# CompVis/unsupervised-part-segmentation

Hardware: AMD Instinct MI355X
Metric: images/sec training (CUB 128x128, 10 parts) (higher is better)
Workload: dtype bf16

## Files before the change

### include/upsparts_hip.h

```cpp
#ifndef UPSPARTS_HIP_H
#define UPSPARTS_HIP_H

#include <stddef.h>
#include <stdint.h>

#ifdef __cplusplus
extern "C" {
#endif

#define UPS_ABI_VERSION 6

enum { UPS_F32 = 0, UPS_BF16 = 1, UPS_F16 = 2 };
enum { UPS_ACT_NONE = 0, UPS_ACT_LRELU = 1, UPS_ACT_RELU = 2, UPS_ACT_ELU = 3 };
enum { UPS_OK = 0, UPS_E_ARG = -1, UPS_E_UNSUPPORTED = -2, UPS_E_LAUNCH = -3 };

int ups_abi_version(void);
void ups_struct_sizes(int64_t out[4]);
const char* ups_last_error(void);

typedef struct {
    int32_t dtype;
    int32_t n, hi, wi;
    int32_t ci;
    int32_t ldi;
// ... 25 lines not shown
    float*       mask_grad;
    const float* mask_view;
    const float* f8_deq;
    const float* f8_scale;
    float*       f8_amax;
    int32_t      f8_e5m2;
    const void*  in_f8;
    void*        out_f8;
    const float* out_f8_scale;
    float*       out_f8_amax;
    int32_t      out_f8_act, out_f8_e5m2;
    int32_t      d2s;
    int32_t      out_act, res_act;
    void*        sign_out;
    const void*  dact_bits;
} ups_conv_desc;

int ups_conv_igemm(const ups_conv_desc* d, void* stream);
int ups_conv_sign_out_written(void);

int ups_weight_prep_d2s(const float* src, int32_t cin_v, int32_t ci_log, int32_t co, int32_t pad_y, int32_t pad_x, int32_t C,
                        void* w, void* stream);

int ups_weight_prep_f8(const float* src, int32_t ntaps, int32_t cin_v, int32_t ci_log, int32_t co, int32_t transpose,
                       void* w_f8, float* deq, void* stream);

typedef struct {
    int32_t dtype;
    int32_t n, hi, wi, ci, ldi;
    int32_t ci_log;
    int32_t cin_v;
    int32_t ho, wo, co, ldo;
    int32_t in_sy, in_sx;
    int32_t ntaps;
    int32_t tap_dy[9], tap_dx[9], tap_w[9];
    int32_t act_in; float act_slope;
    int32_t splitk;
// ... 250 lines not shown
```

### unsupervised-part-segmentation_amd/csrc/common.h

```cpp
#pragma once
#include <hip/hip_runtime.h>
#include <stdint.h>
#include <stdio.h>
#include <type_traits>

#include "../../include/upsparts_hip.h"
#include "env.h"

typedef __bf16 bf16;
typedef __attribute__((ext_vector_type(8))) __bf16 bf16x8;
typedef _Float16 f16;
typedef __attribute__((ext_vector_type(8))) _Float16 f16x8;
typedef __attribute__((ext_vector_type(2))) _Float16 f16x2;
typedef __attribute__((ext_vector_type(4))) short s16x4;
typedef __attribute__((ext_vector_type(4))) float f32x4;
typedef __attribute__((ext_vector_type(16))) float f32x16;

void ups_set_error(const char* fmt, ...);

extern thread_local int g_ups_sign_written;

struct UpsPerDevice {
    unsigned long long bits = 0;
    static int cur() { int d = 0; (void)hipGetDevice(&d); return d & 63; }
// ... 233 lines not shown

__device__ inline float block_sum_256(float v, float* smem4) {
    v = wave_sum(v);
    const int lane = threadIdx.x & 63, wid = threadIdx.x >> 6;
    __syncthreads();
    if (lane == 0) smem4[wid] = v;
    __syncthreads();
    return smem4[0] + smem4[1] + smem4[2] + smem4[3];
}

__device__ __forceinline__ void ups_amax_slot(float* slot, float m) {
    if (m > __builtin_nontemporal_load(slot)) atomicMax((unsigned*)slot, __float_as_uint(m));
}

static inline int ups_cdiv(long long a, long long b) { return (int)((a + b - 1) / b); }
```

### unsupervised-part-segmentation_amd/csrc/conv3x3_patch.hip

```cpp
#include <stdlib.h>

#include "common.h"

namespace {

constexpr int TS = 16;
constexpr int PW = TS + 2;
constexpr int PPIX = PW * PW;
constexpr int RS = 80;
constexpr int PWP = 20;
constexpr int APX = 64;
constexpr int A_BYTES = PW * PWP * APX;
__device__ __forceinline__ int a_swz(int px) { return (px >> 2) & 3; }
__device__ __forceinline__ int a_swz16(int px) { return ((px >> 2) & 1) << 1; }
template <typename T> __device__ __forceinline__ int a_swz_t(int px) { return sizeof(T) == 2 ? a_swz16(px) : a_swz(px); }

template <int V> struct IC { static constexpr int value = V; };

struct PatchK {
    int n, h, w, ci, ldi, co, co_fill, ldo, ldr, ldd, act_in, out_f32, dact_kind, has_ctab;
    float act_slope;
    unsigned long long tap_off, tap_wi;
    const void* in; const void* wgt; void* out;
    const float* bias; const float* coord_tab; const void* res; const void* dact;
    unsigned char* sign_out; const unsigned char* dact_bits;
    const unsigned* mask; float* mask_grad; const float* mask_view;
    int mask_B, mask_P;
    unsigned m_ntn, m_parts, m_tx, m_ty;
    const float* f8_deq; const float* f8_scale; float* f8_amax;
    int f8_e5m2;
    const unsigned char* in_f8; unsigned char* out_f8; const float* out_f8_scale; float* out_f8_amax;
    int out_f8_act, out_f8_e5m2;
    int d2s, d2s_shift;
    int taps_static;
    int out_act, res_act;
    int res_patch;
    int sgn_off;
    int sgn_res;
};

__device__ __forceinline__ int fast_div(int n, int d, unsigned m) {
    if (d == 1) return n;
    return m ? (int)__umulhi((unsigned)n, m) : n / d;
}
static inline unsigned div_magic(long long n_max, int d) {
    if (d <= 1 || n_max * d >= (1ll << 32)) return 0u;
    return (unsigned)(((1ull << 32) + (unsigned)d - 1) / (unsigned)d);
}
// ... 49 lines not shown
                        acc[i][2 * jh + jj] = __builtin_amdgcn_mfma_f32_16x16x32_fp8_bf8(fb[step & 1][jj][1], fa[i][1], acc[i][2 * jh + jj], 0, 0, 0);
                    } else if constexpr (F8 == 1) {
                        acc[i][2 * jh + jj] = __builtin_amdgcn_mfma_f32_16x16x32_fp8_fp8(fb[step & 1][jj][0], fa[i][0], acc[i][2 * jh + jj], 0, 0, 0);
                        acc[i][2 * jh + jj] = __builtin_amdgcn_mfma_f32_16x16x32_fp8_fp8(fb[step & 1][jj][1], fa[i][1], acc[i][2 * jh + jj], 0, 0, 0);
                    } else if constexpr (sizeof(T) == 2 && !__is_same(T, bf16)) {
                        acc[i][2 * jh + jj] = __builtin_amdgcn_mfma_f32_16x16x32_f16(fb[step & 1][jj], fa[i], acc[i][2 * jh + jj], 0, 0, 0);
                    } else {
                        acc[i][2 * jh + jj] = __builtin_amdgcn_mfma_f32_16x16x32_bf16(fb[step & 1][jj], fa[i], acc[i][2 * jh + jj], 0, 0, 0);
                    }
            __builtin_amdgcn_s_setprio(0);
            if (jh + 1 == NP && t + 1 < 3) fetch_a(t + 1);
        }
    }
}

typedef __attribute__((ext_vector_type(8))) int i32x8v;
template <int TM16, int TN16, int ROWB, int ABYTES, int BHALF, bool E5M2, int BBUFS>
__device__ __forceinline__ void f8s_tap(const unsigned char* A, const unsigned char* B, int at, f32x4v (&acc)[TM16][TN16]) {
    typedef __attribute__((ext_vector_type(4))) int i32x4v;
    i32x8v fa[TM16], fb[BBUFS];
    auto cat = [](i32x4v lo, i32x4v hi) __attribute__((always_inline)) -> i32x8v {
        return __builtin_shufflevector(lo, hi, 0, 1, 2, 3, 4, 5, 6, 7);
    };
    auto fetch_b = [&](int j, int slot) __attribute__((always_inline)) {
        fb[slot] = cat(*(const i32x4v*)(B + j * (16 * 64)), *(const i32x4v*)(B + BHALF + j * (16 * 64)));
    };
    fetch_b(0, 0);
#pragma unroll
    for (int i = 0; i < TM16; ++i) fa[i] = cat(*(const i32x4v*)(A + at + i * ROWB), *(const i32x4v*)(A + ABYTES + at + i * ROWB));
#pragma unroll
// ... 38 lines not shown
                                                                     acc[i][j], 0, 0, 0);
    }
};

template <typename T, int BN, int OCC, int SUB, int F8 = 0, bool PRE = false, int TAPS = 0, bool DMAP = false, bool CSTD = false>
__global__ __launch_bounds__(512, 2 * OCC) void conv3x3_patch_kernel(const PatchK p, const int tiles_x, const int tiles_y,
                                                                 const int ntn, const int kchunks, const int nblocks) {
    constexpr int EPC = Chunk<T>::N;
    constexpr int BK = 4 * EPC;
    constexpr int BKA = F8 ? 64 : BK;
    constexpr bool F8S = F8 >= 3;
    constexpr int F8K = F8S ? F8 - 2 : F8;
    static_assert(!F8 || (sizeof(T) == 2 && SUB == TS && (OCC == 1 || PRE)), "fp8 operands: bf16 tensors, one tile per image; two blocks per CU only with a pre-quantised input");
    static_assert(!F8S || (PRE && OCC == 2 && BN >= 64 && TAPS == 0 && !DMAP), "block-scaled fp8: pre-quantised input, two blocks per CU");
    static_assert(!PRE || F8, "a pre-quantised input implies fp8 operands");
    constexpr int WN = (BN == 32) ? 1 : 2;
    constexpr int WM = 8 / WN;
    constexpr int TM = 256 / WM / 32;
    constexpr int TN = BN / WN / 32;
    constexpr int B_BYTES = 3 * BN * RS;
    constexpr int NB = (3 * BN * 4 + 511) / 512;
    constexpr int HALF_OFF = (sizeof(T) == 2) ? 16 : 32;
    constexpr int G = TS / SUB;
    constexpr int PR = G * (SUB + 2);
    constexpr int PWPS = (PR + 3) / 4 * 4;
    constexpr int ABY = PR * PWPS * APX;
    static_assert(SUB == 16 || OCC == 1, "multi-image tiles run one block per CU");

    extern __shared__ __attribute__((aligned(16))) unsigned char smem[];
    unsigned char* Abuf = smem;
// ... 217 lines not shown
    const int r = lane & 31, hh = lane >> 5;
    const int ty_l = (wm * TM * 2) + (r >> 4), tx_l = r & 15;
    const int py_l = ty_l + 2 * (ty_l / SUB) * (SUB < TS ? 1 : 0), px_l = tx_l + 2 * (tx_l / SUB) * (SUB < TS ? 1 : 0);
    const int a_lane_off = (py_l * PWPS + px_l) * APX;
    const int b_lane_off = (wn * TN * 32 + r) * RS + hh * HALF_OFF;
    const int p16 = lane & 15, q16 = lane >> 4;
    const int px_l16 = p16 + 2 * (p16 / SUB) * (SUB < TS ? 1 : 0);
    const int a_lane16 = px_l16 * APX;
    int arow16[TM16];
#pragma unroll
    for (int i = 0; i < TM16; ++i) {
        const int ty = wm * TM16 + i;
        arow16[i] = (ty + 2 * (ty / SUB) * (SUB < TS ? 1 : 0)) * PWPS * APX;
    }

    const int total = 3 * kchunks;
    if constexpr (sizeof(T) == 2) {
        constexpr int BST = 3 * BN * 64;
        constexpr int NJ = 3 * BN * 4 / 64;
        constexpr int NW = (NJ + 7) / 8;
        constexpr bool CHUNKST = (SUB < TS || (CSTD && DMAP && SUB == TS)) && BN <= 64 && F8 == 0 && OCC == 1;
        constexpr int NST = (OCC == 2) ? 2 : (CHUNKST ? 6 : 3);
        constexpr int FRAG_BUFS = (BN == 128) ? 1 : 2;
        unsigned char* Bst = smem + (((kchunks == 1 && SUB == TS) || OCC == 2) ? 1 : 2) * ABY;
        const int boff16 = p16 * 64 + ((q16 ^ a_swz16(p16)) << 4);
        int d_tl[NW];
        unsigned d_off[NW];
#pragma unroll
        for (int q = 0; q < NW; ++q) {
            const int j = (wid + 8 * q) % NJ;
            const int pos = j * 64 + lane, row = pos >> 2, slot = pos & 3;
            const int tl = (j * 16) / BN, rl = row - tl * BN;
            const int c = min(nt * BN + rl, p.co - 1);
            d_tl[q] = tl;
            d_off[q] = (unsigned)(c * BK + (slot ^ a_swz16(row)) * 8) * 2u;
        }
        const unsigned smem_lds = (unsigned)(unsigned long long)(__attribute__((address_space(3))) unsigned char*)smem;
        auto dma_w = [&](int it) __attribute__((always_inline)) {
            const int cc = it / 3, g = it - cc * 3;
            unsigned char* stg = Bst + (it % NST) * BST;
#pragma unroll
            for (int q = 0; q < NW; ++q) {
                const int j = (wid + 8 * q) % NJ;
                const int wslice = TAPS != 0 ? 3 * g + d_tl[q] : p_w(p.tap_wi, 3 * g + d_tl[q]);
                const T* slab = w + ((long long)wslice * kchunks + cc) * p.co * BK;
                const unsigned lds_dst = __builtin_amdgcn_readfirstlane(smem_lds + (unsigned)(stg + j * 1024 - smem));
                asm volatile("s_mov_b32 m0, %0\n\ts_nop 0\n\tglobal_load_lds_dwordx4 %1, %2"
                             :: "s"(lds_dst), "v"(d_off[q]), "s"(slab) : "memory", "m0");
            }
        };
        const unsigned char* __restrict__ in_b = (const unsigned char*)(in + (long long)origin * p.ldi);
        auto dma_patch = [&](int cc, int boff = 0) __attribute__((always_inline)) {
            if constexpr (DMAP) {
                const unsigned char* base = in_b + cc * 64;
#pragma unroll
                for (int q = 0; q < 3; ++q) {
                    if (wid + 8 * q >= (PW * PWPS + 15) / 16) continue;
                    const unsigned lds_dst = __builtin_amdgcn_readfirstlane(smem_lds + (unsigned)(boff + (wid + 8 * q) * 1024));
                    asm volatile("s_mov_b64 exec, %0\n\ts_mov_b32 m0, %1\n\ts_nop 0\n\tglobal_load_lds_dwordx4 %2, %3\n\ts_mov_b64 exec, -1"
                                 :: "s"(pd_mask[q]), "s"(lds_dst), "v"(pd_off[q]), "s"(base) : "memory", "m0");
                }
            }
        };
        const int swx0 = a_lane16 + ((q16 ^ a_swz16(px_l16 + 0)) << 4);
        const int swx1 = a_lane16 + ((q16 ^ a_swz16(px_l16 + 1)) << 4);
        const int swx2 = a_lane16 + ((q16 ^ a_swz16(px_l16 + 2)) << 4);
        constexpr int CPW = TN16 / 2 > 0 ? TN16 / 2 : 1;
        const int rp_first = nt * (BN / 32) + wn * CPW;
        const int rp_lane = ((px_l16 + 1) * APX) + ((((q16 >> 1)) ^ a_swz16(px_l16 + 1)) << 4) + (q16 & 1) * 8;
        constexpr bool RP2 = DMAP && SUB == TS && TN16 >= 2 && TAPS == 2 && BN == 128 && F8 == 0 && __is_same(T, bf16);
        const unsigned char* S1 = smem + p.sgn_off;
        const float rp2_inv = (RP2 && p.res_patch == 2) ? 1.f / dact_ns : 1.f;
        auto add_res_patch = [&](const unsigned char* A, int cc) __attribute__((always_inline)) {
            if constexpr (DMAP && SUB == TS && TN16 >= 2) {
                const int c2 = cc - rp_first;
                if (p.res_patch && c2 >= 0 && c2 < CPW) {
                    int ln = lane;
                    if constexpr (RP2) asm volatile("" : "+v"(ln));
                    const int sg_lane = (ln & 15) * (BN / 8) + (ln >> 5), sg_sh = (ln >> 2) & 4;
#pragma unroll
                    for (int jh = 0; jh < CPW; ++jh) {
// ... 94 lines not shown
            const unsigned char* row = p.dact_bits + (((long long)img_pm * p.h + yy) * p.w + xx) * (p.ldd >> 3) + boff;
            if (yy < p.h && xx < p.w) {
                if (RP2 || (SG_BPP >= 8 && rem >= 8)) sgn_v = *(const uint2*)row;
                else if (rem >= 4) sgn_v.x = *(const unsigned*)row;
            }
        }
        if constexpr (DMAP) dma_patch(0);
        else { load_patch(0); store_patch(Abuf); }
        dma_w(0);
        if (sgn_on && sgn_px < 256) {
            if constexpr (SG_BPP >= 8) *(uint2*)(smem + p.sgn_off + sgn_px * SG_BPP + 8 * sgn_hf) = sgn_v;
            else *(unsigned*)(smem + p.sgn_off + sgn_px * SG_BPP) = sgn_v.x;
        }
        if (OCC != 2 && total > 1) dma_w(1);
        const bool one_shot = OCC != 2 && kchunks == 1;
        if (one_shot || CHUNKST) dma_w(2);
        asm volatile("s_waitcnt vmcnt(0)" ::: "memory");
        __syncthreads();
        if (one_shot) {
            add_res_patch(Abuf, 0);
#pragma unroll
            for (int g = 0; g < 3; ++g) {
                const unsigned char* B = Bst + g * BST + (wn * TN * 32) * 64 + boff16;
                if constexpr (TAPS != 0) {
                    const int po0 = ((TAPS == 1 ? g : 2 - g) * PWPS + (TAPS == 1 ? 0 : 2)) * APX;
                    bf16_taps16<T, TM16, TN16, (SUB == TS ? PWPS * APX : 0), F8>(Abuf, B, arow16, po0, po0 + (TAPS == 1 ? APX : -APX),
                                            po0 + (TAPS == 1 ? 2 * APX : -2 * APX), TAPS == 1 ? swx0 : swx2, swx1, TAPS == 1 ? swx2 : swx0,
                                            BN * 64, acc16);
                } else {
                    const int dx0 = p_dx(p.tap_off, 3 * g) + 1, dx1 = p_dx(p.tap_off, 3 * g + 1) + 1, dx2 = p_dx(p.tap_off, 3 * g + 2) + 1;
                    const int po0 = ((p_dy(p.tap_off, 3 * g) + 1) * PWPS + dx0) * APX;
                    const int po1 = ((p_dy(p.tap_off, 3 * g + 1) + 1) * PWPS + dx1) * APX;
                    const int po2 = ((p_dy(p.tap_off, 3 * g + 2) + 1) * PWPS + dx2) * APX;
// ... 492 lines not shown
        "conv3x3_patch_kernel", (epi > shmem_max ? epi : shmem_max) + sgn_bytes, dim3(nblocks), dim3(512), shmem, s, kk, tiles_x, tiles_y, ntn,
        kchunks, nblocks);
}

template <typename T, int SUB>
int launch_small(const PatchK& k, hipStream_t s) {
    const int tiles = k.n / ((TS / SUB) * (TS / SUB));
    if (k.co_fill > 64 && tiles * ups_cdiv(k.co_fill, 128) >= 192) return launch_bn<T, 128, 1, SUB>(k, s);
    if (k.co_fill > 32 && tiles * ups_cdiv(k.co_fill, 64) >= 128) return launch_bn<T, 64, 1, SUB>(k, s);
    return launch_bn<T, 32, 1, SUB>(k, s);
}

template <typename T, int BN, int OCC>
int launch_v(const PatchK& k, hipStream_t s) {
    const bool dmap = k.act_in == UPS_ACT_NONE && !k.mask && !k.mask_grad && k.ci % 32 == 0;
    if (dmap) {
        if (k.taps_static == 1) return launch_bn<T, BN, OCC, TS, 0, false, 1, true>(k, s);
        if (k.taps_static == 2) return launch_bn<T, BN, OCC, TS, 0, false, 2, true>(k, s);
    }
    if (k.taps_static == 1 && BN == 128 && OCC == 2) return launch_bn<T, BN, OCC, TS, 0, false, (BN == 128 && OCC == 2) ? 1 : 0>(k, s);
    return launch_bn<T, BN, OCC, TS>(k, s);
}

template <typename T>
int launch_t(const PatchK& k, hipStream_t s) {
    if (k.h == 8) return launch_small<T, 8>(k, s);
    if (k.h == 4) return launch_small<T, 4>(k, s);
    if constexpr (sizeof(T) == 2) {
      if constexpr (__is_same(T, bf16)) {
        if (k.f8_deq && k.in_f8) {
// ... 19 lines not shown
            }
            if (k.co_fill > 64) return launch_bn<T, 128, 1, TS, 1>(k, s);
            if (k.co_fill > 32) return launch_bn<T, 64, 1, TS, 1>(k, s);
            return launch_bn<T, 32, 1, TS, 1>(k, s);
        }
      }
        const int tiles = k.n * ((k.w + TS - 1) / TS) * ((k.h + TS - 1) / TS);
        if (k.co_fill > 64 && k.ci > 32) {
            if (!k.out_f8_amax && tiles * ups_cdiv(k.co_fill, 128) >= 512) return launch_v<T, 128, 2>(k, s);
            if (tiles * ups_cdiv(k.co_fill, 64) >= 512) return launch_v<T, 64, 2>(k, s);
            {
                const bool dmap = k.act_in == UPS_ACT_NONE && !k.mask && !k.mask_grad && k.ci % 32 == 0;
                if (dmap && !k.out_f8_amax && k.ci >= 128 && tiles * ups_cdiv(k.co_fill, 128) <= 256) {
                    if (k.taps_static == 1) return launch_bn<T, 64, 1, TS, 0, false, 1, true, true>(k, s);
                    if (k.taps_static == 2) return launch_bn<T, 64, 1, TS, 0, false, 2, true, true>(k, s);
                }
            }
            return launch_v<T, 128, 1>(k, s);
        }
        if (k.co_fill > 32) {
            if (k.co_fill > 64 && tiles * ups_cdiv(k.co_fill, 128) >= 512) {
                if (k.out_f8_amax) return launch_bn<T, 128, 2, TS>(k, s);
                return launch_v<T, 128, 2>(k, s);
            }
            return (k.ci > 32 && tiles * ups_cdiv(k.co_fill, 64) >= 512) ? launch_v<T, 64, 2>(k, s) : launch_v<T, 64, 1>(k, s);
        }
        return launch_v<T, 32, 1>(k, s);
    } else {
        if (k.co_fill > 64) return launch_bn<T, 128, 1, TS>(k, s);
        if (k.co_fill > 32) return launch_bn<T, 64, 1, TS>(k, s);
// ... 32 lines not shown
        seen[(dy + 1) * 3 + dx + 1] = true;
    }
    for (int t = 0; t < 9; ++t) if (!seen[t]) return 1;
    if (d->coord_tab) {
        for (int t = 0; t < 9; ++t) if (d->tap_dy[t] != t / 3 - 1 || d->tap_dx[t] != t % 3 - 1) return 1;
    }
    PatchK k;
    k.mask = d->mask_bits; k.mask_grad = d->mask_grad; k.mask_view = d->mask_view;
    k.f8_deq = d->f8_deq; k.f8_scale = d->f8_scale; k.f8_amax = d->f8_amax; k.f8_e5m2 = d->f8_e5m2;
    k.in_f8 = (const unsigned char*)d->in_f8; k.out_f8 = (unsigned char*)d->out_f8; k.out_f8_scale = d->out_f8_scale;
    k.out_f8_amax = d->out_f8_amax; k.out_f8_act = d->out_f8_act; k.out_f8_e5m2 = d->out_f8_e5m2;
    if (d->in_f8 && (!d->f8_deq || d->co_fill <= 32)) return 1;
    if ((d->out_f8 || d->out_f8_amax) && (d->dtype != UPS_BF16 || small || d->out_f32 || (d->ldo & 7) || (d->co_fill & 7) || d->mask_grad ||
                                          !d->out_f8_amax || (d->out_f8 && !d->out_f8_scale)))
        return 1;
    k.d2s = 0; k.d2s_shift = 0;
    if (d->d2s) {
        if (d->dtype != UPS_BF16 || small || (d->hi % TS) || (d->wi % TS) || d->d2s < 8 || (d->d2s & (d->d2s - 1)) ||
            d->co != 4 * d->d2s || d->co_fill != d->co || d->out_f32 || (d->ldo & 7) || d->mask_bits || d->mask_grad ||
            d->coord_tab || d->bias || d->f8_deq)
            return 1;
        k.d2s = 1;
        while ((1 << k.d2s_shift) < d->d2s) ++k.d2s_shift;
    }
    if (d->f8_deq) {
        if (d->dtype != UPS_BF16 || small || (d->hi % TS) || (d->wi % TS) || d->ci % 64 || d->mask_bits || d->mask_grad ||
            !d->f8_scale || (!d->f8_amax && !d->in_f8))
            return 1;
    }
    k.mask_B = 0; k.mask_P = 1;
    if (d->mask_bits || d->mask_grad) {
        if (d->dtype != UPS_BF16 || small || d->mask_batch <= 0 || d->n % d->mask_batch) return 1;
        if (d->mask_bits && d->mask_grad) return 1;
        k.mask_B = d->mask_batch; k.mask_P = d->n / d->mask_batch;
        if (k.mask_P > 32) return 1;
        if (d->mask_grad && (!d->mask_view || d->out_f32 || (d->ldo & 7) || (d->co_fill & 7) || d->co_fill > 32 || d->res || d->dact)) return 1;
    }
    k.n = d->n; k.h = d->hi; k.w = d->wi; k.ci = d->ci; k.ldi = d->ldi; k.co = d->co; k.co_fill = d->co_fill;
    k.ldo = d->ldo; k.ldr = d->ldr; k.ldd = d->ldd; k.act_in = d->act_in; k.out_f32 = d->out_f32;
    k.dact_kind = d->dact_kind; k.has_ctab = d->coord_tab != nullptr; k.act_slope = d->act_slope;
    k.in = d->in; k.wgt = d->w; k.out = d->out; k.bias = d->bias; k.coord_tab = d->coord_tab; k.res = d->res; k.dact = d->dact;
    k.sign_out = ups_conv3x3_patch_signs(d) ? (unsigned char*)d->sign_out : nullptr;
    k.dact_bits = (d->dact && ups_conv3x3_patch_signs(d) && (d->ldd & 7) == 0) ? (const unsigned char*)d->dact_bits : nullptr;
    bool fwd = true, flip = true;
    {
        for (int t = 0; t < 9; ++t) {
            if (d->tap_w[t] != t) fwd = flip = false;
            if (d->tap_dy[t] != t / 3 - 1 || d->tap_dx[t] != t % 3 - 1) fwd = false;
            if (d->tap_dy[t] != 1 - t / 3 || d->tap_dx[t] != 1 - t % 3) flip = false;
        }
        k.taps_static = fwd ? 1 : (flip ? 2 : 0);
    }
    k.out_act = d->out_act; k.res_act = d->res_act;
    {
        k.res_patch = d->res && d->res == d->in && d->ldr == d->ldi && d->ci == d->co_fill && d->co == d->co_fill && d->ci % 32 == 0 &&
                      d->dtype != UPS_F32 && !small && !d->dact && !d->mask_bits && !d->mask_grad && !d->d2s && !d->f8_deq && !d->out_f32 &&
                      d->act_in == UPS_ACT_NONE &&
                      (fwd || flip);
        if (!k.res_patch && d->res && d->res == d->in && d->ldr == d->ldi && d->ci == d->co_fill && d->co == d->co_fill &&
            d->ci % 32 == 0 && d->dtype == UPS_BF16 && !small && d->dact && k.dact_bits && d->dact_kind == UPS_ACT_LRELU && d->act_slope > 0.f &&
            (d->ldd & 63) == 0 && (((uintptr_t)k.dact_bits) & 7) == 0 && !d->mask_bits && !d->mask_grad && !d->d2s && !d->f8_deq && !d->out_f32 &&
            !d->res_act && d->act_in == UPS_ACT_NONE && flip && !fwd)
            k.res_patch = 2;
    }
    if ((d->out_act || d->res_act) && (d->mask_grad || d->d2s)) return 1;
    if (d->out_act && (d->out_f8 || d->out_f8_amax) && d->out_f8_act != UPS_ACT_NONE) return 1;
// ... 11 lines not shown
```

### unsupervised-part-segmentation_amd/csrc/conv_aux.hip

```cpp
#include "common.h"

namespace {

template <typename T>
__global__ void weight_prep_kernel(const float* __restrict__ src, int ntaps, int cin_v, int ci_log, int co,
                                   T* __restrict__ wf, int ci_pad, T* __restrict__ wd, int drows, int dk) {
    constexpr int BK = 64 / (int)sizeof(T);
    const int kcf = (ci_pad + BK - 1) / BK, kcd = (dk + BK - 1) / BK;
    const long long nf = wf ? (long long)ntaps * kcf * co * BK : 0;
    const long long nd = wd ? (long long)ntaps * kcd * drows * BK : 0;
    for (long long idx = (long long)blockIdx.x * blockDim.x + threadIdx.x; idx < nf + nd;
         idx += (long long)gridDim.x * blockDim.x) {
        if (idx < nf) {
            const int kk = (int)(idx % BK);
            long long t = idx / BK;
            const int c = (int)(t % co); t /= co;
            const int kc = (int)(t % kcf), tap = (int)(t / kcf);
            const int k = kc * BK + kk;
            const float v = k < ci_log ? src[((long long)tap * cin_v + k) * co + c] : 0.f;
            st_from_float<T>(wf + idx, v);
        } else {
            const long long j = idx - nf;
            const int kk = (int)(j % BK);
            long long t = j / BK;
// ... 379 lines not shown
}

namespace {
__global__ __launch_bounds__(256) void weight_prep_d2s_kernel(const float* __restrict__ src, int cin_v, int ci_log, int co,
                                                              int pad_y, int pad_x, int C, int kc, uint4* __restrict__ w,
                                                              long long total) {
    const long long i = (long long)blockIdx.x * 256 + threadIdx.x;
    if (i >= total) return;
    const int piece = (int)(i & 3);
    long long r = i >> 2;
    const int row = (int)(r % (4 * C)); r /= 4 * C;
    const int k = (int)(r % kc);
    const int t9 = (int)(r / kc);
    const int dy = t9 / 3 - 1, dx = t9 % 3 - 1;
    const int cls = row / C, c = row - cls * C, py = cls >> 1, px = cls & 1;
    const int rr = py + pad_y - 2 * dy, ss = px + pad_x - 2 * dx;
    float f[8];
#pragma unroll
    for (int e = 0; e < 8; ++e) {
        const int kk = k * 32 + piece * 8 + e;
        f[e] = (rr >= 0 && rr < 3 && ss >= 0 && ss < 3 && c < ci_log && kk < co)
                   ? src[((long long)(rr * 3 + ss) * cin_v + c) * co + kk] : 0.f;
    }
    w[i] = Chunk<bf16>::pack(f);
}
}

extern "C" int ups_weight_prep_d2s(const float* src, int32_t cin_v, int32_t ci_log, int32_t co, int32_t pad_y, int32_t pad_x,
                                   int32_t C, void* w, void* stream) {
    UPS_CHECK_ARG(src && w && ci_log >= 1 && cin_v >= ci_log && co >= 1 && C >= ci_log && C >= 8 && (C & (C - 1)) == 0);
    const int kc = (co + 31) / 32;
    const long long total = 9ll * kc * 4 * C * 4;
    hipLaunchKernelGGL(weight_prep_d2s_kernel, dim3((unsigned)((total + 255) / 256)), dim3(256), 0, (hipStream_t)stream, src, cin_v,
                       ci_log, co, pad_y, pad_x, C, kc, (uint4*)w, total);
    UPS_LAUNCH_CHECK();
    return UPS_OK;
}

extern "C" int64_t ups_prep_item_blocks(const ups_prep_item* item_host, int32_t dtype) {
    if (!item_host) return -1;
    return (prep_elems(*item_host, dtype == UPS_F32 ? 16 : 32) + 255) / 256;
}

extern "C" int ups_weight_prep_batch(const ups_prep_item* items, const int64_t* block_prefix, int32_t n_items,
                                     int64_t total_blocks, int32_t dtype, void* stream) {
    UPS_CHECK_ARG(items && block_prefix && n_items >= 1 && total_blocks >= 1 && total_blocks < 0x7fffffffLL);
    if (dtype == UPS_F32)
        hipLaunchKernelGGL(weight_prep_batch_kernel<float>, dim3((unsigned)ups_cdiv(total_blocks, PREP_CPB)), dim3(256), 0, (hipStream_t)stream,
                           items, (const long long*)block_prefix, n_items, (long long)total_blocks);
    else if (dtype == UPS_F16)
        hipLaunchKernelGGL(weight_prep_batch_kernel<f16>, dim3((unsigned)ups_cdiv(total_blocks, PREP_CPB)), dim3(256), 0, (hipStream_t)stream,
                           items, (const long long*)block_prefix, n_items, (long long)total_blocks);
// ... 79 lines not shown
```

### unsupervised-part-segmentation_amd/lib.py

```python
import ctypes as C
import os

import torch

from . import switches as SW

_HERE = os.path.dirname(os.path.abspath(__file__))
LIB_PATH = SW.value("UPS_LIB") or os.path.join(_HERE, "csrc", "libupsparts_hip.so")

ABI_VERSION = 6
F32, BF16, F16 = 0, 1, 2
ACT_NONE, ACT_LRELU, ACT_RELU, ACT_ELU = 0, 1, 2, 3
ACT = {None: ACT_NONE, "leaky_relu": ACT_LRELU, "relu": ACT_RELU, "elu": ACT_ELU}


class UpsError(RuntimeError):
    pass


class ConvDesc(C.Structure):
    _fields_ = [("dtype", C.c_int32), ("n", C.c_int32), ("hi", C.c_int32), ("wi", C.c_int32), ("ci", C.c_int32),
                ("ldi", C.c_int32), ("ho", C.c_int32), ("wo", C.c_int32), ("co", C.c_int32), ("co_fill", C.c_int32),
                ("ldo", C.c_int32), ("out_h", C.c_int32), ("out_w", C.c_int32), ("out_sy", C.c_int32),
                ("out_sx", C.c_int32), ("out_oy", C.c_int32), ("out_ox", C.c_int32), ("in_sy", C.c_int32),
                ("in_sx", C.c_int32), ("ntaps", C.c_int32), ("kh", C.c_int32), ("kw", C.c_int32),
                ("tap_dy", C.c_int32 * 9), ("tap_dx", C.c_int32 * 9), ("tap_w", C.c_int32 * 9),
                ("act_in", C.c_int32), ("act_slope", C.c_float), ("out_f32", C.c_int32), ("dact_kind", C.c_int32),
                ("ldr", C.c_int32), ("ldd", C.c_int32),
                ("in_", C.c_void_p), ("w", C.c_void_p), ("out", C.c_void_p), ("bias", C.c_void_p),
                ("coord_tab", C.c_void_p), ("res", C.c_void_p), ("dact", C.c_void_p),
                ("workspace", C.c_void_p), ("workspace_bytes", C.c_size_t),
                ("mask_bits", C.c_void_p), ("mask_batch", C.c_int32), ("mask_grad", C.c_void_p), ("mask_view", C.c_void_p),
                ("f8_deq", C.c_void_p), ("f8_scale", C.c_void_p), ("f8_amax", C.c_void_p), ("f8_e5m2", C.c_int32),
                ("in_f8", C.c_void_p), ("out_f8", C.c_void_p), ("out_f8_scale", C.c_void_p), ("out_f8_amax", C.c_void_p),
                ("out_f8_act", C.c_int32), ("out_f8_e5m2", C.c_int32), ("d2s", C.c_int32),
                ("out_act", C.c_int32), ("res_act", C.c_int32), ("sign_out", C.c_void_p), ("dact_bits", C.c_void_p)]


class WgradDesc(C.Structure):
    _fields_ = [("dtype", C.c_int32), ("n", C.c_int32), ("hi", C.c_int32), ("wi", C.c_int32), ("ci", C.c_int32),
                ("ldi", C.c_int32), ("ci_log", C.c_int32), ("cin_v", C.c_int32), ("ho", C.c_int32), ("wo", C.c_int32),
                ("co", C.c_int32), ("ldo", C.c_int32), ("in_sy", C.c_int32), ("in_sx", C.c_int32), ("ntaps", C.c_int32),
                ("tap_dy", C.c_int32 * 9), ("tap_dx", C.c_int32 * 9), ("tap_w", C.c_int32 * 9),
                ("act_in", C.c_int32), ("act_slope", C.c_float), ("splitk", C.c_int32),
                ("in_", C.c_void_p), ("dout", C.c_void_p), ("grad", C.c_void_p), ("grad_bias", C.c_void_p),
                ("workspace", C.c_void_p), ("mask_bits", C.c_void_p), ("mask_batch", C.c_int32), ("in_f16", C.c_int32),
                ("dout_f8", C.c_void_p), ("dout_f8_scale", C.c_void_p), ("in_f8_scale", C.c_void_p), ("in_f8_amax", C.c_void_p)]


class PriorDesc(C.Structure):
    _fields_ = [("n", C.c_int32), ("h", C.c_int32), ("w", C.c_int32), ("P", C.c_int32), ("view", C.c_int32),
# ... 19 lines not shown
                ("k", C.c_int32), ("n", C.c_int32)]


_lib = None

_I, _L, _F, _P, _Z = C.c_int32, C.c_int64, C.c_float, C.c_void_p, C.c_size_t
_SIGS = {
    "ups_abi_version": ([], C.c_int),
    "ups_struct_sizes": ([C.POINTER(C.c_int64)], None),
    "ups_conv_igemm": ([C.POINTER(ConvDesc), _P], C.c_int),
    "ups_conv_wgrad_plan": ([C.POINTER(WgradDesc), C.POINTER(_I), C.POINTER(_Z)], C.c_int),
    "ups_conv_wgrad": ([C.POINTER(WgradDesc), _P], C.c_int),
    "ups_weight_prep": ([_P, _I, _I, _I, _I, _I, _P, _I, _P, _I, _I, _P], C.c_int),
    "ups_weight_prep_f8": ([_P, _I, _I, _I, _I, _I, _P, _P, _P], C.c_int),
    "ups_weight_prep_d2s": ([_P, _I, _I, _I, _I, _I, _I, _P, _P], C.c_int),
    "ups_prep_item_blocks": ([C.POINTER(PrepItem), _I], C.c_int64),
    "ups_weight_prep_batch": ([_P, _P, _I, _L, _I, _P], C.c_int),
    "ups_coord_table": ([_P, _I, _I, _I, _I, C.POINTER(_I), C.POINTER(_I), _I, _I, _F, _F, _P, _P], C.c_int),
    "ups_batch_sum": ([_P, _I, _I, _L, _I, _I, _P, _P], C.c_int),
    "ups_coord_wgrad": ([_P, _I, _I, _I, _I, _I, _I, _I, C.POINTER(_I), C.POINTER(_I), _I, _I, _F, _F, _I, _P, _P, _P, _P], C.c_int),
    "ups_col_sum": ([_P, _I, _L, _I, _I, _P, _P, _P], C.c_int),
    "ups_deconv_prep": ([_P, _P, _I, _I, _I, _I, _P, _I, _P, _P, _P, _P, _I, _I, _P], C.c_int),
    "ups_deconv3x3_s2_fwd": ([_P, _I, _I, _I, _I, _I, _I, _P, _P, _P, _I, _I, _P, _P], C.c_int),
    "ups_deconv_bias_coord_grad": ([_P, _I, _I, _I, _I, _I, _I, _I, _P, _P, _P, _I, _P], C.c_int),
    "ups_deconv_wn_bwd": ([_P, _P, _P, _P, _I, _I, _I, _P, _P, _P], C.c_int),
    "ups_bilinear2x_fwd": ([_P, _P, _I, _I, _I, _I, _I, _P], C.c_int),
    "ups_bilinear2x_bwd": ([_P, _P, _I, _I, _I, _I, _I, _P], C.c_int),
    "ups_depth_to_space": ([_P, _P, _I, _I, _I, _I, _I, _I, _I, _I, _P], C.c_int),
    "ups_nearest2x": ([_P, _P, _I, _I, _I, _I, _I, _I, _P], C.c_int),
    "ups_crop_fwd": ([_P, _P, _I, _I, _I, _I, _I, _I, _I, _P, _P], C.c_int),
# ... 158 lines not shown
```

### unsupervised-part-segmentation_amd/ops.py

```python
import ctypes as C
import os

import torch

from . import lib as L
from . import switches as SW


def round8(c):
    return (c + 7) // 8 * 8


def same_geometry(size, k, stride):
    out = -(-size // stride)
    pad_total = max((out - 1) * stride + k - size, 0)
    return out, pad_total // 2


class _Workspace(object):

    def __init__(self):
        self.bufs = {}

    def get(self, nbytes, device):
# ... 644 lines not shown
        g_hard = torch.empty((n, hi, wi, n_parts), dtype=torch.float32, device=x.device)
        gx = None
        n_img = n * n_parts
    else:
        gx = torch.empty_like(x)
        n_img = n
    k, st = layer.k, layer.stride
    _, pby = same_geometry(hi, k, st)
    _, pbx = same_geometry(wi, k, st)
    cd2s = layer.d2s_channels(x) if mask_view is None else 0
    if cd2s:
        d = _conv_desc(dcode, g, (n, ho, wo, round8(layer.co), g.shape[-1]), layer.prepared_d2s(hi, wi)["w"], gx,
                       (ho, wo, 4 * cd2s, 4 * cd2s, ldi), ([t // 3 - 1 for t in range(9)], [t % 3 - 1 for t in range(9)], range(9)),
                       3, 3, layer.slope, lattice=(hi, wi, 1, 0, 0))
        _attach_dgrad(d, layer, x, x_bits, res)
        d.d2s = cd2s
        _launch_conv(d, layer)
        return gx
    classes = [(0, 0)] if st == 1 else [(py, px) for py in range(st) for px in range(st)]
    for (py, px) in classes:
        lat_h = (hi - py + st - 1) // st
        lat_w = (wi - px + st - 1) // st
        if lat_h <= 0 or lat_w <= 0:
            continue
        dy, dx, tw = [], [], []
        for r in range(k):
            if (py + pby - r) % st:
                continue
            for s in range(k):
                if (px + pbx - s) % st:
                    continue
# ... 1270 lines not shown
```

Baseline: 2155.

## Skip structurally zero taps in depth-to-space strided dgrad conv

Adds a live-tap mask for the depth-to-space form of the strided convolution's input gradient, computed from the padding. The patch kernel gets a dedicated path that runs only two of the three tap rows and skips 32-column MFMA steps whose weights are zero for every parity class. The mask is specialised at compile time through a small set of dispatch cases. This removes MFMA and weight-DMA work on zero weights, at the cost of more kernel instantiations and a new pipeline schedule with its own barrier and wait logic.

Result: no change. 2174, median of 6 (+0.9%).

```diff
diff --git a/include/upsparts_hip.h b/include/upsparts_hip.h
--- a/include/upsparts_hip.h
+++ b/include/upsparts_hip.h
@@ -63,6 +63,7 @@
     int32_t      out_act, res_act;
     void*        sign_out;
     const void*  dact_bits;
+    int32_t      d2s_pad_y, d2s_pad_x;
 } ups_conv_desc;
 
 int ups_conv_igemm(const ups_conv_desc* d, void* stream);
@@ -70,6 +71,7 @@
 
 int ups_weight_prep_d2s(const float* src, int32_t cin_v, int32_t ci_log, int32_t co, int32_t pad_y, int32_t pad_x, int32_t C,
                         void* w, void* stream);
+uint64_t ups_d2s_live(int32_t pad_y, int32_t pad_x);
 
 int ups_weight_prep_f8(const float* src, int32_t ntaps, int32_t cin_v, int32_t ci_log, int32_t co, int32_t transpose,
                        void* w_f8, float* deq, void* stream);
diff --git a/unsupervised-part-segmentation_amd/csrc/common.h b/unsupervised-part-segmentation_amd/csrc/common.h
--- a/unsupervised-part-segmentation_amd/csrc/common.h
+++ b/unsupervised-part-segmentation_amd/csrc/common.h
@@ -271,3 +271,16 @@
 }
 
 static inline int ups_cdiv(long long a, long long b) { return (int)((a + b - 1) / b); }
+
+__host__ __device__ inline int ups_d2s_fwd_tap(int par, int pad, int d) {
+    const int r = par + pad - 2 * d;
+    return (r >= 0 && r < 3) ? r : -1;
+}
+static inline unsigned long long ups_d2s_live_mask(int pad_y, int pad_x) {
+    unsigned long long m = 0;
+    for (int t9 = 0; t9 < 9; ++t9)
+        for (int cls = 0; cls < 4; ++cls)
+            if (ups_d2s_fwd_tap(cls >> 1, pad_y, t9 / 3 - 1) >= 0 && ups_d2s_fwd_tap(cls & 1, pad_x, t9 % 3 - 1) >= 0)
+                m |= 1ull << (t9 * 4 + cls);
+    return m;
+}
diff --git a/unsupervised-part-segmentation_amd/csrc/conv3x3_patch.hip b/unsupervised-part-segmentation_amd/csrc/conv3x3_patch.hip
--- a/unsupervised-part-segmentation_amd/csrc/conv3x3_patch.hip
+++ b/unsupervised-part-segmentation_amd/csrc/conv3x3_patch.hip
@@ -32,6 +32,7 @@
     const unsigned char* in_f8; unsigned char* out_f8; const float* out_f8_scale; float* out_f8_amax;
     int out_f8_act, out_f8_e5m2;
     int d2s, d2s_shift;
+    unsigned long long d2s_live;
     int taps_static;
     int out_act, res_act;
     int res_patch;
@@ -111,6 +112,44 @@
     }
 }
 
+template <int TM16, int TN16, int ROWB, unsigned LM>
+__device__ __forceinline__ void bf16_taps16_live(const unsigned char* A, const unsigned char* B, const int (&arow)[TM16],
+                                                 int po0, int po1, int sw0, int sw1, int b_tap_stride, f32x4v (&acc)[TM16][TN16]) {
+    typedef bf16x8 frag_t;
+    constexpr int NP = TN16 / 2, NS = 2 * NP;
+    static_assert(LM != 0 && LM < (1u << NS) && ROWB > 0, "a non-empty set of steps of two taps, one tile per image");
+    frag_t fa[TM16], fb[2][2];
+    auto fetch_a = [&](int t) __attribute__((always_inline)) {
+        const unsigned char* at = A + (arow[0] + (t == 0 ? po0 : po1)) + (t == 0 ? sw0 : sw1);
+#pragma unroll
+        for (int i = 0; i < TM16; ++i) fa[i] = *(const frag_t*)(at + i * ROWB);
+    };
+    auto fetch_b = [&](int t, int jh, int slot) __attribute__((always_inline)) {
+#pragma unroll
+        for (int jj = 0; jj < 2; ++jj) fb[slot][jj] = *(const frag_t*)(B + t * b_tap_stride + (2 * jh + jj) * (16 * 64));
+    };
+    constexpr int S0 = __builtin_ctz(LM);
+    fetch_a(S0 / NP);
+    fetch_b(S0 / NP, S0 % NP, 0);
+#pragma unroll
+    for (int step = 0; step < NS; ++step) {
+        if (!((LM >> step) & 1u)) continue;
+        const int ord = __builtin_popcount(LM & ((1u << step) - 1u));
+        const unsigned rest = LM >> (step + 1);
+        const int nx = rest ? step + 1 + __builtin_ctz(rest) : NS;
+        const int jh = step % NP;
+        if (nx < NS) fetch_b(nx / NP, nx % NP, (ord + 1) & 1);
+        __builtin_amdgcn_s_setprio(1);
+#pragma unroll
+        for (int i = 0; i < TM16; ++i)
+#pragma unroll
+            for (int jj = 0; jj < 2; ++jj)
+                acc[i][2 * jh + jj] = __builtin_amdgcn_mfma_f32_16x16x32_bf16(fb[ord & 1][jj], fa[i], acc[i][2 * jh + jj], 0, 0, 0);
+        __builtin_amdgcn_s_setprio(0);
+        if (nx < NS && nx / NP != step / NP) fetch_a(nx / NP);
+    }
+}
+
 typedef __attribute__((ext_vector_type(8))) int i32x8v;
 template <int TM16, int TN16, int ROWB, int ABYTES, int BHALF, bool E5M2, int BBUFS>
 __device__ __forceinline__ void f8s_tap(const unsigned char* A, const unsigned char* B, int at, f32x4v (&acc)[TM16][TN16]) {
@@ -179,6 +218,9 @@
     static_assert(!F8 || (sizeof(T) == 2 && SUB == TS && (OCC == 1 || PRE)), "fp8 operands: bf16 tensors, one tile per image; two blocks per CU only with a pre-quantised input");
     static_assert(!F8S || (PRE && OCC == 2 && BN >= 64 && TAPS == 0 && !DMAP), "block-scaled fp8: pre-quantised input, two blocks per CU");
     static_assert(!PRE || F8, "a pre-quantised input implies fp8 operands");
+    constexpr bool D2S = TAPS == 3;
+    constexpr int RPC = D2S ? 2 : 3;
+    static_assert(!D2S || (__is_same(T, bf16) && F8 == 0 && SUB == TS), "d2s: bf16, one tile per image");
     constexpr int WN = (BN == 32) ? 1 : 2;
     constexpr int WM = 8 / WN;
     constexpr int TM = 256 / WM / 32;
@@ -426,13 +468,13 @@
         arow16[i] = (ty + 2 * (ty / SUB) * (SUB < TS ? 1 : 0)) * PWPS * APX;
     }
 
-    const int total = 3 * kchunks;
+    const int total = RPC * kchunks;
     if constexpr (sizeof(T) == 2) {
         constexpr int BST = 3 * BN * 64;
-        constexpr int NJ = 3 * BN * 4 / 64;
+        constexpr int NJ = RPC * BN * 4 / 64;
         constexpr int NW = (NJ + 7) / 8;
         constexpr bool CHUNKST = (SUB < TS || (CSTD && DMAP && SUB == TS)) && BN <= 64 && F8 == 0 && OCC == 1;
-        constexpr int NST = (OCC == 2) ? 2 : (CHUNKST ? 6 : 3);
+        constexpr int NST = (OCC == 2) ? 2 : (CHUNKST ? 2 * RPC : 3);
         constexpr int FRAG_BUFS = (BN == 128) ? 1 : 2;
         unsigned char* Bst = smem + (((kchunks == 1 && SUB == TS) || OCC == 2) ? 1 : 2) * ABY;
         const int boff16 = p16 * 64 + ((q16 ^ a_swz16(p16)) << 4);
@@ -449,7 +491,7 @@
         }
         const unsigned smem_lds = (unsigned)(unsigned long long)(__attribute__((address_space(3))) unsigned char*)smem;
         auto dma_w = [&](int it) __attribute__((always_inline)) {
-            const int cc = it / 3, g = it - cc * 3;
+            const int cc = it / RPC, g = it - cc * RPC;
             unsigned char* stg = Bst + (it % NST) * BST;
 #pragma unroll
             for (int q = 0; q < NW; ++q) {
@@ -477,6 +519,21 @@
         const int swx0 = a_lane16 + ((q16 ^ a_swz16(px_l16 + 0)) << 4);
         const int swx1 = a_lane16 + ((q16 ^ a_swz16(px_l16 + 1)) << 4);
         const int swx2 = a_lane16 + ((q16 ^ a_swz16(px_l16 + 2)) << 4);
+        unsigned d2s_lm[2] = {0u, 0u};
+        if constexpr (D2S) {
+#pragma unroll
+            for (int g = 0; g < 2; ++g)
+#pragma unroll
+                for (int t = 0; t < 2; ++t)
+#pragma unroll
+                    for (int jh = 0; jh < TN16 / 2; ++jh) {
+                        const int col0 = nt * BN + (wn * (TN16 / 2) + jh) * 32;
+                        const int c0 = col0 >> p.d2s_shift, c1 = min((col0 + 31) >> p.d2s_shift, 3);
+                        const unsigned span = ((2u << c1) - 1u) & ~((1u << c0) - 1u);
+                        if ((unsigned)(p.d2s_live >> ((3 * g + t) * 4)) & span) d2s_lm[g] |= 1u << (t * (TN16 / 2) + jh);
+                    }
+            d2s_lm[0] = __builtin_amdgcn_readfirstlane(d2s_lm[0]); d2s_lm[1] = __builtin_amdgcn_readfirstlane(d2s_lm[1]);
+        }
         constexpr int CPW = TN16 / 2 > 0 ? TN16 / 2 : 1;
         const int rp_first = nt * (BN / 32) + wn * CPW;
         const int rp_lane = ((px_l16 + 1) * APX) + ((((q16 >> 1)) ^ a_swz16(px_l16 + 1)) << 4) + (q16 & 1) * 8;
@@ -601,9 +658,105 @@
         }
         if (OCC != 2 && total > 1) dma_w(1);
         const bool one_shot = OCC != 2 && kchunks == 1;
-        if (one_shot || CHUNKST) dma_w(2);
+        if ((one_shot || CHUNKST) && !D2S) dma_w(2);
         asm volatile("s_waitcnt vmcnt(0)" ::: "memory");
         __syncthreads();
+        if constexpr (D2S) {
+        auto run = [&](auto lm0c, auto lm1c) __attribute__((always_inline)) {
+            auto row = [&](const unsigned char* A, const unsigned char* B, auto gc) __attribute__((always_inline)) {
+                constexpr int g = decltype(gc)::value;
+                constexpr unsigned LM = g == 0 ? (unsigned)decltype(lm0c)::value : (unsigned)decltype(lm1c)::value;
+                if constexpr (LM != 0u)
+                    bf16_taps16_live<TM16, TN16, PWPS * APX, LM>(A, B, arow16, g * PWPS * APX, g * PWPS * APX + APX, swx0, swx1, BN * 64, acc16);
+            };
+            auto sync_all = [&]() __attribute__((always_inline)) {
+                asm volatile("s_waitcnt vmcnt(0)" ::: "memory");
+                asm volatile("s_waitcnt lgkmcnt(0)" ::: "memory");
+                __builtin_amdgcn_s_barrier();
+            };
+            const unsigned char* Bw = Bst + (wn * TN * 32) * 64 + boff16;
+            if (one_shot) {
+                row(Abuf, Bw, IC<0>{});
+                row(Abuf, Bw + BST, IC<1>{});
+                asm volatile("s_waitcnt lgkmcnt(0)" ::: "memory");
+                __builtin_amdgcn_s_barrier();
+            } else if constexpr (OCC == 2) {
+                for (int cc = 0; cc < kchunks; ++cc) {
+                    const bool more = cc + 1 < kchunks;
+                    dma_w(2 * cc + 1);
+                    row(Abuf, Bw, IC<0>{});
+                    sync_all();
+                    if (more) {
+                        if constexpr (!DMAP) load_patch(cc + 1);
+                        dma_w(2 * cc + 2);
+                    }
+                    row(Abuf, Bw + BST, IC<1>{});
+                    if (more) {
+                        asm volatile("s_waitcnt lgkmcnt(0)" ::: "memory");
+                        __builtin_amdgcn_s_barrier();
+                        if constexpr (DMAP) dma_patch(cc + 1);
+                        else store_patch(Abuf);
+                    }
+                    sync_all();
+                }
+            } else if constexpr (CHUNKST) {
+                for (int cc = 0; cc < kchunks; ++cc) {
+                    const bool more = cc + 1 < kchunks;
+                    if (more) {
+                        if constexpr (DMAP) dma_patch(cc + 1, ((cc + 1) & 1) * ABY);
+                        else load_patch(cc + 1);
+                        dma_w(2 * cc + 2); dma_w(2 * cc + 3);
+                    }
+                    const unsigned char* A = Abuf + (cc & 1) * ABY;
+                    row(A, Bw + ((2 * cc) % NST) * BST, IC<0>{});
+                    row(A, Bw + ((2 * cc + 1) % NST) * BST, IC<1>{});
+                    if constexpr (!DMAP) { if (more) store_patch(Abuf + ((cc + 1) & 1) * ABY); }
+                    sync_all();
+                }
+            } else {
+                auto wait_next = [&](bool in_flight) __attribute__((always_inline)) {
+                    if (in_flight) {
+                        if (NW == 2) asm volatile("s_waitcnt vmcnt(2)" ::: "memory");
+                        else asm volatile("s_waitcnt vmcnt(1)" ::: "memory");
+                    } else {
+                        asm volatile("s_waitcnt vmcnt(0)" ::: "memory");
+                    }
+                    asm volatile("s_waitcnt lgkmcnt(0)" ::: "memory");
+                    __builtin_amdgcn_s_barrier();
+                };
+                static_assert(NW <= 2, "two taps of at most 128 rows: at most two DMA instructions per wave and stage");
+                for (int cc = 0; cc < kchunks; ++cc) {
+                    const bool more = cc + 1 < kchunks;
+                    const unsigned char* A = Abuf + (cc & 1) * ABY;
+                    if (more) {
+                        if constexpr (DMAP) dma_patch(cc + 1, ((cc + 1) & 1) * ABY);
+                        else load_patch(cc + 1);
+                        dma_w(2 * cc + 2);
+                    }
+                    row(A, Bw + ((2 * cc) % 3) * BST, IC<0>{});
+                    wait_next(more);
+                    if (more) dma_w(2 * cc + 3);
+                    row(A, Bw + ((2 * cc + 1) % 3) * BST, IC<1>{});
+                    if constexpr (!DMAP) { if (more) store_patch(Abuf + ((cc + 1) & 1) * ABY); }
+                    wait_next(more);
+                }
+            }
+        };
+        const unsigned lm0 = d2s_lm[0], lm1 = d2s_lm[1];
+        if constexpr (TN16 == 4) {
+            if (lm1 == 0xDu && lm0 == 0xDu) run(IC<0xD>{}, IC<0xD>{});
+            else if (lm1 == 0xDu && lm0 == 0u) run(IC<0>{}, IC<0xD>{});
+            else if (lm1 == 0xCu && lm0 == 0xCu) run(IC<0xC>{}, IC<0xC>{});
+            else if (lm1 == 0xCu && lm0 == 0u) run(IC<0>{}, IC<0xC>{});
+            else if (lm1 == 0xFu && lm0 == 0u) run(IC<0>{}, IC<0xF>{});
+            else run(IC<0xF>{}, IC<0xF>{});
+        } else {
+            if (lm1 == 0x2u && lm0 == 0x2u) run(IC<2>{}, IC<2>{});
+            else if (lm1 == 0x2u && lm0 == 0u) run(IC<0>{}, IC<2>{});
+            else if (lm1 == 0x3u && lm0 == 0u) run(IC<0>{}, IC<3>{});
+            else run(IC<3>{}, IC<3>{});
+        }
+        } else
         if (one_shot) {
             add_res_patch(Abuf, 0);
 #pragma unroll
@@ -1126,6 +1279,12 @@
 template <typename T, int BN, int OCC>
 int launch_v(const PatchK& k, hipStream_t s) {
     const bool dmap = k.act_in == UPS_ACT_NONE && !k.mask && !k.mask_grad && k.ci % 32 == 0;
+    if constexpr (__is_same(T, bf16)) {
+        if (k.taps_static == 3) {
+            if (dmap) return launch_bn<T, BN, OCC, TS, 0, false, 3, true>(k, s);
+            return launch_bn<T, BN, (BN == 128 ? 1 : OCC), TS, 0, false, 3, false>(k, s);
+        }
+    }
     if (dmap) {
         if (k.taps_static == 1) return launch_bn<T, BN, OCC, TS, 0, false, 1, true>(k, s);
         if (k.taps_static == 2) return launch_bn<T, BN, OCC, TS, 0, false, 2, true>(k, s);
@@ -1175,6 +1334,7 @@
                 if (dmap && !k.out_f8_amax && k.ci >= 128 && tiles * ups_cdiv(k.co_fill, 128) <= 256) {
                     if (k.taps_static == 1) return launch_bn<T, 64, 1, TS, 0, false, 1, true, true>(k, s);
                     if (k.taps_static == 2) return launch_bn<T, 64, 1, TS, 0, false, 2, true, true>(k, s);
+                    if constexpr (__is_same(T, bf16)) { if (k.taps_static == 3) return launch_bn<T, 64, 1, TS, 0, false, 3, true, true>(k, s); }
                 }
             }
             return launch_v<T, 128, 1>(k, s);
@@ -1237,7 +1397,7 @@
     if ((d->out_f8 || d->out_f8_amax) && (d->dtype != UPS_BF16 || small || d->out_f32 || (d->ldo & 7) || (d->co_fill & 7) || d->mask_grad ||
                                           !d->out_f8_amax || (d->out_f8 && !d->out_f8_scale)))
         return 1;
-    k.d2s = 0; k.d2s_shift = 0;
+    k.d2s = 0; k.d2s_shift = 0; k.d2s_live = 0;
     if (d->d2s) {
         if (d->dtype != UPS_BF16 || small || (d->hi % TS) || (d->wi % TS) || d->d2s < 8 || (d->d2s & (d->d2s - 1)) ||
             d->co != 4 * d->d2s || d->co_fill != d->co || d->out_f32 || (d->ldo & 7) || d->mask_bits || d->mask_grad ||
@@ -1245,6 +1405,10 @@
             return 1;
         k.d2s = 1;
         while ((1 << k.d2s_shift) < d->d2s) ++k.d2s_shift;
+        if ((d->d2s_pad_y | d->d2s_pad_x) & ~1) return 1;
+        k.d2s_live = ups_d2s_live_mask(d->d2s_pad_y, d->d2s_pad_x);
+        for (int t9 = 0; t9 < 9; ++t9)
+            if ((t9 / 3 == 2 || t9 % 3 == 2) && ((k.d2s_live >> (4 * t9)) & 15ull)) return 1;
     }
     if (d->f8_deq) {
         if (d->dtype != UPS_BF16 || small || (d->hi % TS) || (d->wi % TS) || d->ci % 64 || d->mask_bits || d->mask_grad ||
@@ -1273,6 +1437,10 @@
             if (d->tap_dy[t] != 1 - t / 3 || d->tap_dx[t] != 1 - t % 3) flip = false;
         }
         k.taps_static = fwd ? 1 : (flip ? 2 : 0);
+        if (d->d2s) {
+            if (!fwd) return 1;
+            k.taps_static = 3;
+        }
     }
     k.out_act = d->out_act; k.res_act = d->res_act;
     {
diff --git a/unsupervised-part-segmentation_amd/csrc/conv_aux.hip b/unsupervised-part-segmentation_amd/csrc/conv_aux.hip
--- a/unsupervised-part-segmentation_amd/csrc/conv_aux.hip
+++ b/unsupervised-part-segmentation_amd/csrc/conv_aux.hip
@@ -417,12 +417,12 @@
     const int t9 = (int)(r / kc);
     const int dy = t9 / 3 - 1, dx = t9 % 3 - 1;
     const int cls = row / C, c = row - cls * C, py = cls >> 1, px = cls & 1;
-    const int rr = py + pad_y - 2 * dy, ss = px + pad_x - 2 * dx;
+    const int rr = ups_d2s_fwd_tap(py, pad_y, dy), ss = ups_d2s_fwd_tap(px, pad_x, dx);
     float f[8];
 #pragma unroll
     for (int e = 0; e < 8; ++e) {
         const int kk = k * 32 + piece * 8 + e;
-        f[e] = (rr >= 0 && rr < 3 && ss >= 0 && ss < 3 && c < ci_log && kk < co)
+        f[e] = (rr >= 0 && ss >= 0 && c < ci_log && kk < co)
                    ? src[((long long)(rr * 3 + ss) * cin_v + c) * co + kk] : 0.f;
     }
     w[i] = Chunk<bf16>::pack(f);
@@ -439,6 +439,8 @@
     UPS_LAUNCH_CHECK();
     return UPS_OK;
 }
+
+extern "C" uint64_t ups_d2s_live(int32_t pad_y, int32_t pad_x) { return ups_d2s_live_mask(pad_y, pad_x); }
 
 extern "C" int64_t ups_prep_item_blocks(const ups_prep_item* item_host, int32_t dtype) {
     if (!item_host) return -1;
diff --git a/unsupervised-part-segmentation_amd/lib.py b/unsupervised-part-segmentation_amd/lib.py
--- a/unsupervised-part-segmentation_amd/lib.py
+++ b/unsupervised-part-segmentation_amd/lib.py
@@ -34,7 +34,8 @@
                 ("f8_deq", C.c_void_p), ("f8_scale", C.c_void_p), ("f8_amax", C.c_void_p), ("f8_e5m2", C.c_int32),
                 ("in_f8", C.c_void_p), ("out_f8", C.c_void_p), ("out_f8_scale", C.c_void_p), ("out_f8_amax", C.c_void_p),
                 ("out_f8_act", C.c_int32), ("out_f8_e5m2", C.c_int32), ("d2s", C.c_int32),
-                ("out_act", C.c_int32), ("res_act", C.c_int32), ("sign_out", C.c_void_p), ("dact_bits", C.c_void_p)]
+                ("out_act", C.c_int32), ("res_act", C.c_int32), ("sign_out", C.c_void_p), ("dact_bits", C.c_void_p),
+                ("d2s_pad_y", C.c_int32), ("d2s_pad_x", C.c_int32)]
 
 
 class WgradDesc(C.Structure):
@@ -84,6 +85,7 @@
     "ups_weight_prep": ([_P, _I, _I, _I, _I, _I, _P, _I, _P, _I, _I, _P], C.c_int),
     "ups_weight_prep_f8": ([_P, _I, _I, _I, _I, _I, _P, _P, _P], C.c_int),
     "ups_weight_prep_d2s": ([_P, _I, _I, _I, _I, _I, _I, _P, _P], C.c_int),
+    "ups_d2s_live": ([_I, _I], C.c_uint64),
     "ups_prep_item_blocks": ([C.POINTER(PrepItem), _I], C.c_int64),
     "ups_weight_prep_batch": ([_P, _P, _I, _L, _I, _P], C.c_int),
     "ups_coord_table": ([_P, _I, _I, _I, _I, C.POINTER(_I), C.POINTER(_I), _I, _I, _F, _F, _P, _P], C.c_int),
diff --git a/unsupervised-part-segmentation_amd/ops.py b/unsupervised-part-segmentation_amd/ops.py
--- a/unsupervised-part-segmentation_amd/ops.py
+++ b/unsupervised-part-segmentation_amd/ops.py
@@ -682,7 +682,7 @@
                        (ho, wo, 4 * cd2s, 4 * cd2s, ldi), ([t // 3 - 1 for t in range(9)], [t % 3 - 1 for t in range(9)], range(9)),
                        3, 3, layer.slope, lattice=(hi, wi, 1, 0, 0))
         _attach_dgrad(d, layer, x, x_bits, res)
-        d.d2s = cd2s
+        d.d2s, d.d2s_pad_y, d.d2s_pad_x = cd2s, pby, pbx
         _launch_conv(d, layer)
         return gx
     classes = [(0, 0)] if st == 1 else [(py, px) for py in range(st) for px in range(st)]
```
